# WWWindrunner/Cross-Modal-Video-Engine

Hardware: AMD Instinct MI355X
Metric: query-video pairs/sec scored + R@1/5/10 parity, MSR-VTT-1kA at 1/8 GPU (higher is better)
Workload: dtype f16

## Files before the change

cross-modal-video-engine_amd/csrc/cmve_internal.h:

```cpp
#pragma once
#include <hip/hip_runtime.h>
#include <hip/hip_ext.h>
#include <stdint.h>
#include <math.h>
#include <string>
#include <algorithm>
#include <type_traits>
#include "../../include/cmve.h"

struct cmve_handle {
  int device;
  hipStream_t stream;
  hipStream_t aux = nullptr;
  hipEvent_t ev[CMVE_MAX_CHUNKS + 2] = {};
  hipEvent_t tev[2 * CMVE_MAX_CHUNKS] = {};
  int last_chunks = 0;
  hipEvent_t eval_ev[CMVE_EVAL_TIMING_SLOTS][4] = {};
  hipEvent_t eval_kev[CMVE_EVAL_TIMING_SLOTS][8] = {};
  bool eval_no_fix[CMVE_EVAL_TIMING_SLOTS] = {};
  bool eval_chained[CMVE_EVAL_TIMING_SLOTS] = {};
  void* scratch = nullptr;
  size_t scratch_bytes = 0;
  void* comm = nullptr;
  int nranks = 1, rank = 0;
// ... 225 lines not shown
      load4d(x + k, v);
#pragma unroll
      for (int c = 0; c < 4; ++c) ss = fma(v[c], v[c], ss);
    }
    return wave_sum(ss);
  }
  for (int64_t k = lane; k < d; k += WAVE) {
    const double v = (double)x[k];
    ss = fma(v, v, ss);
  }
  return wave_sum(ss);
}
__device__ __forceinline__ double row_inv_norm(double ss, double eps, int flags) {
  const double nrm = sqrt(ss);
  return (flags & CMVE_PACK_RAW) ? 1.0 : (eps > 0.0 ? 1.0 / fmax(nrm, eps) : 1.0 / nrm);
}

struct PackAcc {
  double e1 = 0.0, e2 = 0.0, e3 = 0.0;
  float e4 = 0.f;
};

__device__ __forceinline__ int xcd_linear(int bid, int total) {
  const int xcd = bid & 7, local = bid >> 3;
  const int q = total >> 3, r = total & 7;
  return (xcd < r ? xcd * (q + 1) : r * (q + 1) + (xcd - r) * q) + local;
}

__device__ __forceinline__ uint16_t lo16_elem(float xf, _Float16 h, float& res) {
  const float d2 = xf - (float)h;
  const uint16_t lo = f2bf(d2);
  res = d2 - bf2f(lo);
  return lo;
}
__device__ __forceinline__ float lo16_bound(double ss_res) {
  return f32_round_up(sqrt(ss_res) * (1.0 + 1e-4) + 5.9605e-8 * (1.0 + 1e-6) + 1e-12);
}
__device__ __forceinline__ _Float16 f16_via_f32(double xh, float& xf) {
  xf = (float)xh;
  asm volatile("" : "+v"(xf));
  return (_Float16)xf;
}

__device__ __forceinline__ void pack_elem(double xh, bool want_f16, uint16_t& h, uint16_t& l, uint16_t& f,
                                          PackAcc& acc) {
  float xf;
  const _Float16 hf16 = f16_via_f32(xh, xf);
  if (want_f16) {
    const double r3 = xh - (double)hf16;
    acc.e3 = fma(r3, r3, acc.e3);
    f = __builtin_bit_cast(uint16_t, hf16);
  }
  h = f2bf(xf);
  const float hf = bf2f(h);
  l = f2bf(xf - hf);
  const double r1 = xh - (double)hf;
  const double r2 = r1 - (double)bf2f(l);
  acc.e1 = fma(r1, r1, acc.e1);
  acc.e2 = fma(r2, r2, acc.e2);
}

typedef unsigned short cmve_u16x4 __attribute__((ext_vector_type(4)));
typedef uint32_t cmve_u32x2 __attribute__((ext_vector_type(2)));

__device__ __forceinline__ void pack_pad_row(uint16_t* hrow, uint16_t* lrow, uint16_t* frow, int64_t d_pad,
                                             int lane) {
  const cmve_u16x4 z = {0, 0, 0, 0};
  for (int64_t k = (int64_t)lane * 4; k < d_pad; k += 256) {
    gst((cmve_u16x4*)(hrow + k), z);
    if (lrow) gst((cmve_u16x4*)(lrow + k), z);
    if (frow) gst((cmve_u16x4*)(frow + k), z);
  }
}

template <typename T>
__device__ __forceinline__ void pack_row_planes(const T* __restrict__ x, int64_t d, int64_t d_pad, bool vec,
                                                double inv, uint16_t* hrow, uint16_t* lrow, uint16_t* frow,
                                                int lane, float& b1, float& b2, float& b3) {
  const bool want_f16 = frow != nullptr;
  PackAcc acc;
  bool done = false;
  if (vec) {
    for (int64_t k = (int64_t)lane * 4; k < d_pad; k += 256) {
      cmve_u16x4 hv = {0, 0, 0, 0}, lv = {0, 0, 0, 0}, fv = {0, 0, 0, 0};
      if (k < d) {
        double e[4];
        load4d(x + k, e);
#pragma unroll
        for (int c = 0; c < 4; ++c) {
          uint16_t h, l, f = 0;
          pack_elem(e[c] * inv, want_f16, h, l, f, acc);
          hv[c] = h;
          lv[c] = l;
          fv[c] = f;
        }
      }
      *(cmve_u16x4*)(hrow + k) = hv;
      if (lrow) *(cmve_u16x4*)(lrow + k) = lv;
      if (frow) *(cmve_u16x4*)(frow + k) = fv;
    }
    done = true;
  }
  if (!done)
    for (int64_t k = lane; k < d_pad; k += WAVE) {
      uint16_t h = 0, l = 0, f = 0;
      if (k < d) pack_elem((double)x[k] * inv, want_f16, h, l, f, acc);
      hrow[k] = h;
      if (lrow) lrow[k] = l;
      if (frow) frow[k] = f;
    }
  const double e1 = wave_sum(acc.e1), e2 = wave_sum(acc.e2), e3 = wave_sum(acc.e3);
  b1 = f32_round_up(sqrt(e1) * (1.0 + 1e-9) + 1e-12);
  b2 = f32_round_up(sqrt(e2) * (1.0 + 1e-9) + 1e-12);
  b3 = f32_round_up(sqrt(e3) * (1.0 + 1e-9) + 1e-12);
}

__device__ __forceinline__ int64_t gt_rank_of(int32_t cnt, double sgt, int64_t n_m) {
  return (sgt != sgt) ? n_m + 1 : (sgt == (double)INFINITY ? n_m : (int64_t)cnt + 1);
}

constexpr int CAND_BUCKET_SHIFT = 8;
struct CandLayout {
  int64_t nb, cap_b;
};
inline CandLayout cand_layout(int64_t g_n_pad, int64_t cap) {
  CandLayout l;
  l.nb = std::max<int64_t>(1, (g_n_pad + (1 << CAND_BUCKET_SHIFT) - 1) >> CAND_BUCKET_SHIFT);
  l.cap_b = cap > l.nb ? (cap - l.nb) / l.nb : 0;
  return l;
}
constexpr int64_t FIXUP_MAX_BUCKETS_PER_XCD = 4096;
constexpr int EVAL_EMAX_SHARDS = 64;

template <typename TA, typename TB, bool LIGHT = false>
__device__ __forceinline__ double wave_cos64(const TA* xa, const TB* xb, double inva, double invb, int64_t d,
                                             int lane) {
  return wave_dot64<TA, TB, LIGHT>(xa, xb, d, lane) * (inva * invb);
}

typedef uint32_t cmve_u32x4 __attribute__((ext_vector_type(4)));
struct L16Frag {
  cmve_u32x4 h0, h1, l0, l1;
};
__device__ __forceinline__ void l16_load(const uint16_t* __restrict__ hrow, const uint16_t* __restrict__ lrow,
                                         int64_t k, L16Frag& f) {
  f.h0 = gld((const cmve_u32x4*)(hrow + k));
  f.h1 = gld((const cmve_u32x4*)(hrow + k + 8));
  f.l0 = gld((const cmve_u32x4*)(lrow + k));
  f.l1 = gld((const cmve_u32x4*)(lrow + k + 8));
}
__device__ __forceinline__ double l16_x(uint32_t hw, uint32_t lw, int half) {
  const uint16_t h = (uint16_t)(hw >> (16 * half));
  const uint32_t l = half ? (lw & 0xffff0000u) : (lw << 16);
  return (double)(float)__builtin_bit_cast(_Float16, h) + (double)__uint_as_float(l);
}
__device__ __forceinline__ double l16_partial(const L16Frag& a, const L16Frag& b, double acc) {
  const uint32_t ah[8] = {a.h0.x, a.h0.y, a.h0.z, a.h0.w, a.h1.x, a.h1.y, a.h1.z, a.h1.w};
  const uint32_t al[8] = {a.l0.x, a.l0.y, a.l0.z, a.l0.w, a.l1.x, a.l1.y, a.l1.z, a.l1.w};
  const uint32_t bh[8] = {b.h0.x, b.h0.y, b.h0.z, b.h0.w, b.h1.x, b.h1.y, b.h1.z, b.h1.w};
  const uint32_t bl[8] = {b.l0.x, b.l0.y, b.l0.z, b.l0.w, b.l1.x, b.l1.y, b.l1.z, b.l1.w};
#pragma unroll
  for (int e = 0; e < 16; ++e)
    acc = fma(l16_x(ah[e >> 1], al[e >> 1], e & 1), l16_x(bh[e >> 1], bl[e >> 1], e & 1), acc);
  return acc;
}
__device__ __forceinline__ void fixup_prefix(const uint64_t* __restrict__ cand, int64_t nb, int64_t cap_b, int xcd,
                                             int G, int64_t nk, int lane, int64_t* pre) {
  const int64_t per = (nk + 63) / 64;
  const int64_t k0 = lane * per, k1 = min(nk, k0 + per);
  if (per <= 4) {
    int64_t v[4];
#pragma unroll
    for (int j = 0; j < 4; ++j) v[j] = (k0 + j < k1) ? min((int64_t)gld(cand + xcd + G * (k0 + j)), cap_b) : 0;
    const int64_t sum = (v[0] + v[1]) + (v[2] + v[3]);
    int64_t incl = sum;
    for (int o = 1; o < 64; o <<= 1) {
      const int64_t t = __shfl_up(incl, o, 64);
      if (lane >= o) incl += t;
    }
    int64_t run = incl - sum;
#pragma unroll
    for (int j = 0; j < 4; ++j)
      if (k0 + j < k1) {
        pre[k0 + j] = run;
        run += v[j];
      }
    if (lane == 63) pre[nk] = incl;
  } else {
    int64_t sum = 0;
    for (int64_t k = k0; k < k1; ++k) sum += min((int64_t)gld(cand + xcd + G * k), cap_b);
    int64_t incl = sum;
    for (int o = 1; o < 64; o <<= 1) {
      const int64_t t = __shfl_up(incl, o, 64);
      if (lane >= o) incl += t;
    }
    int64_t run = incl - sum;
    for (int64_t k = k0; k < k1; ++k) {
      pre[k] = run;
      run += min((int64_t)gld(cand + xcd + G * k), cap_b);
    }
    if (lane == 63) pre[nk] = incl;
  }
}

template <typename TQ, typename TG, bool PREFETCH = false, bool DYN_PRE = false, bool LIGHT = false>
__device__ __forceinline__ void fixup_walk(const TQ* __restrict__ qraw, int64_t ldq,
                                                    const double* __restrict__ qinv, const TG* __restrict__ graw,
                                                    int64_t ldg, const double* __restrict__ ginv, int64_t d,
                                                    const double* __restrict__ row_sgt,
                                                    const double* __restrict__ col_sgt, int* __restrict__ row_cnt,
                                                    int* __restrict__ col_cnt, const uint64_t* __restrict__ cand,
                                                    int64_t nb, int64_t cap_b, bool flat = false) {
  int64_t* pre;
  if constexpr (DYN_PRE) {
    extern __shared__ int64_t fix_dyn_pre[];
    pre = fix_dyn_pre;
  } else {
    __shared__ int64_t fix_pre[FIXUP_MAX_BUCKETS_PER_XCD + 1];
    pre = fix_pre;
  }
  const int lane = threadIdx.x & 63, wave = threadIdx.x >> 6;
  const int G = flat ? 1 : 8;
  const int xcd = flat ? 0 : (blockIdx.x & 7);
  const int64_t nk = xcd < nb ? (nb - xcd + G - 1) / G : 0;
  if (wave == 0) fixup_prefix(cand, nb, cap_b, xcd, G, nk, lane, pre);
  __syncthreads();
  const int64_t total = pre[nk];
  const int nw = (int)(blockDim.x >> 6);
  const int64_t stride = (int64_t)(gridDim.x / G) * nw;
  int64_t k = 0;
  auto entry = [&](int64_t cc) -> uint64_t {
    if (cc >= total) return 0ull;
    if (pre[k + 1] <= cc) {
      int64_t lo = k + 1, hi = nk - 1;
      while (lo < hi) {
        const int64_t mid = (lo + hi + 1) >> 1;
        if (pre[mid] <= cc) lo = mid;
        else hi = mid - 1;
      }
      k = lo;
    }
    return gld(cand + nb + (xcd + G * k) * cap_b + (cc - pre[k]));
  };
  const int64_t c0 = (int64_t)(blockIdx.x / G) * nw + wave;
  uint64_t u_next = entry(c0);
  for (int64_t c = c0; c < total;) {
    const uint64_t u = u_next;
    c += stride;
    u_next = entry(c);
    const int64_t i = (int64_t)(u & 0x7fffffffull);
    const int64_t j = (int64_t)((u >> 31) & 0x7fffffffull);
    uint32_t flags = (uint32_t)(u >> 62);
    if (!flags) continue;
    double rs = 0.0, cs = 0.0;
    if (PREFETCH) {
      rs = ((flags & 1u) && row_sgt) ? gld(row_sgt + i) : 0.0;
      cs = ((flags & 2u) && col_sgt) ? gld(col_sgt + j) : 0.0;
    }
    const double s = wave_cos64<TQ, TG, LIGHT>(qraw + i * ldq, graw + j * ldg, gld(qinv + i), gld(ginv + j), d, lane);
    if (lane == 0) {
      if ((flags & 1u) && row_sgt && s > (PREFETCH ? rs : gld(row_sgt + i))) gadd(row_cnt + i, 1);
      if ((flags & 2u) && col_sgt && s > (PREFETCH ? cs : gld(col_sgt + j))) gadd(col_cnt + j, 1);
    }
  }
}

__device__ __forceinline__ uint32_t topk_key(float f) {
  const uint32_t u = __float_as_uint(f);
  if (f != f) return 0u;
  return (u & 0x80000000u) ? ~u : (u | 0x80000000u);
}
__device__ __forceinline__ float topk_key_inv(uint32_t k) {
  return __uint_as_float((k & 0x80000000u) ? (k & 0x7fffffffu) : ~k);
}

__host__ __device__ __forceinline__ double score_error_bound(double ea, double eb, int64_t d_pad, int mode) {
  const double n = (double)d_pad * (33.0 / 32.0) * (mode == CMVE_SIM_BF16X3 ? 3.0 : 1.0);
  const double u = 1.0 / 8388608.0;
  const double gamma = n * u / (1.0 - n * u);
  return ea + (1.0 + ea) * eb + gamma * (1.0 + ea) * (1.0 + eb) + 1e-12;
}

inline const float* mode_err(const cmve_rows_t* r, int mode) {
  return mode == CMVE_SIM_BF16 ? r->err_hi : (mode == CMVE_SIM_BF16X3 ? r->err_hilo : r->err_h16);
}
__host__ __device__ __forceinline__ int mode_slot(int mode) { return mode; }

}
```

cross-modal-video-engine_amd/csrc/sim.hip:

```cpp
#include <algorithm>
#include <vector>

#include <hip/hip_ext.h>

#include "cmve_internal.h"

#ifndef CMVE_SIM_GN
#define CMVE_SIM_GN 8
#endif
#ifndef CMVE_EVAL_DBG
#define CMVE_EVAL_DBG 0
#endif
namespace cmve {

typedef __bf16 bf16x8_t __attribute__((ext_vector_type(8)));
typedef _Float16 f16x8_t __attribute__((ext_vector_type(8)));
typedef short s16x8_t __attribute__((ext_vector_type(8)));
typedef float f32x4_t __attribute__((ext_vector_type(4)));
typedef __attribute__((address_space(3))) void lds_void_t;

constexpr int BK = 64;
constexpr int EPI_STORE = 0, EPI_RANK = 1, EPI_LINEAR = 2, EPI_TOPK = 3, EPI_BIAS = 4;
constexpr bool epi_thr(int e) { return e == EPI_RANK || e == EPI_TOPK; }

struct SimArgs {
  const uint16_t* qhi;
  const uint16_t* qlo;
  const uint16_t* ghi;
  const uint16_t* glo;
  int64_t ldk;
  int nq, ng;
  int nblk_m, nblk_n;
  int nk;
  int nk0;
  int gn;
  const float* bias;
  const float* bn_scale;
  const float* bn_shift;
  const float* resid;
  int64_t ldr;
  int relu;
  void* out;
  int64_t ldo;
  float alpha, beta;
  int out_f64;
  const float* row_hi;
  const float* row_lo;
  const float* col_hi;
  const float* col_lo;
  int* row_cnt;
  int* col_cnt;
  unsigned long long* cand;
  long long cand_cap;
  unsigned long long* cand_count;
  unsigned long long* bucket_cnt;
  long long cap_b;
  int thr_gt;
  const double* row_sgt;
  const double* col_sgt;
  const float* q_err;
  const float* g_err;
  const unsigned* q_emax;
  const unsigned* g_emax;
  unsigned long long* dbg_stamps;
  int tile_buckets;
  int nbn64;
  const int* row_gt1;
  const int* col_gt1;
  int fix_inline;
  int q_f64, g_f64;
  const void* q_raw;
  const void* g_raw;
  int64_t q_ld, g_ld, d;
  const double* q_inv;
  const double* g_inv;
  const uint16_t* q_lo16;
  const uint16_t* g_lo16;
  const float* q_el;
  const float* g_el;
  unsigned* l3_count;
  unsigned long long* l3;
  int l3_cap;
};

__device__ __forceinline__ void tile_grouped(int L, int nblk_m, int nblk_n, int GN, int& bm, int& bn);
__device__ __forceinline__ void tile_of_block(int bid, int nblk_m, int nblk_n, int GN, int& bm, int& bn) {
  tile_grouped(xcd_linear(bid, nblk_m * nblk_n), nblk_m, nblk_n, GN, bm, bn);
}
__device__ __forceinline__ void tile_grouped(int L, int nblk_m, int nblk_n, int GN, int& bm, int& bn) {
  const int group = L / (GN * nblk_m);
  const int within = L - group * (GN * nblk_m);
  const int gn = min(GN, nblk_n - group * GN);
  bm = within / gn;
  bn = group * GN + (within - bm * gn);
}

__host__ __device__ constexpr int lds_swz(int r) { return r & 7; }

__device__ __forceinline__ uint32_t stage_lane_off(int64_t ldk, int lane) {
  constexpr int CPR = BK / 8;
  const int r = lane / CPR, c = lane % CPR;
  return (uint32_t)(((int64_t)r * ldk + (c ^ lds_swz(r)) * 8) * 2);
}

template <int ROWS, int NW>
__device__ __forceinline__ void stage_plane(const uint16_t* __restrict__ src, int64_t ldk, int row0, int k0,
                                            char* lds_plane, int wave, uint32_t loff) {
  constexpr int RPI = 64 / (BK / 8);
  constexpr int PER_WAVE = ROWS / RPI / NW;
  static_assert(PER_WAVE * RPI * NW == ROWS, "plane rows must split evenly over the waves");
  static_assert(lds_swz(RPI) == 0 && lds_swz(RPI - 1) == lds_swz(2 * RPI - 1), "swizzle period");
  const char* blk = (const char*)(src + ((int64_t)row0 + wave * PER_WAVE * RPI) * ldk + k0);
#pragma unroll
  for (int it = 0; it < PER_WAVE; ++it)
    __builtin_amdgcn_global_load_lds((const void*)(blk + (int64_t)it * RPI * ldk * 2 + loff),
                                     (lds_void_t*)(lds_plane + (wave * PER_WAVE + it) * 1024), 16, 0, 0);
}

__device__ __forceinline__ s16x8_t read_frag(const char* plane, int row, int chunk) {
  return *(const s16x8_t*)(plane + row * (BK * 2) + ((chunk ^ lds_swz(row)) << 4));
}

__device__ __forceinline__ void lds_add_u32_async(int* p, int v) {
  const uint32_t addr = (uint32_t)(uintptr_t)(__attribute__((address_space(3))) int*)p;
  asm volatile("ds_add_u32 %0, %1" ::"v"(addr), "v"(v) : "memory");
}

__device__ __forceinline__ uint32_t row_sum16(uint32_t v) {
  v += (uint32_t)__builtin_amdgcn_update_dpp(0, (int)v, 0xB1, 0xF, 0xF, false);
  v += (uint32_t)__builtin_amdgcn_update_dpp(0, (int)v, 0x4E, 0xF, 0xF, false);
  v += (uint32_t)__builtin_amdgcn_update_dpp(0, (int)v, 0x141, 0xF, 0xF, false);
  v += (uint32_t)__builtin_amdgcn_update_dpp(0, (int)v, 0x140, 0xF, 0xF, false);
  return v;
}

template <int R>
__device__ __forceinline__ uint32_t row4_count_bits(float s0, float s1, float s2, float s3, float hi, float lo,
                                                    uint32_t& u) {
  uint32_t c, b0, b1, b2, b3;
  unsigned long long m0, m1, m2, m3, l0, l1, l2, l3, cc;
  asm("v_cmp_gt_f32_e64 %[m0], %[s0], %[hi]\n\t"
      "v_cmp_gt_f32_e64 %[m1], %[s1], %[hi]\n\t"
      "v_cmp_gt_f32_e64 %[m2], %[s2], %[hi]\n\t"
      "v_cmp_gt_f32_e64 %[m3], %[s3], %[hi]\n\t"
      "v_cmp_ge_f32_e64 %[l0], %[s0], %[lo]\n\t"
      "v_cmp_ge_f32_e64 %[l1], %[s1], %[lo]\n\t"
      "v_cmp_ge_f32_e64 %[l2], %[s2], %[lo]\n\t"
      "v_cmp_ge_f32_e64 %[l3], %[s3], %[lo]\n\t"
      "v_cndmask_b32_e64 %[c], 0, 1, %[m0]\n\t"
      "v_addc_co_u32_e64 %[c], %[cc], %[c], 0, %[m1]\n\t"
      "v_addc_co_u32_e64 %[c], %[cc], %[c], 0, %[m2]\n\t"
      "v_addc_co_u32_e64 %[c], %[cc], %[c], 0, %[m3]\n\t"
      "s_andn2_b64 %[l0], %[l0], %[m0]\n\t"
      "s_andn2_b64 %[l1], %[l1], %[m1]\n\t"
      "s_andn2_b64 %[l2], %[l2], %[m2]\n\t"
      "s_andn2_b64 %[l3], %[l3], %[m3]\n\t"
      "v_cndmask_b32_e64 %[b0], 0, 1, %[l0]\n\t"
      "v_cndmask_b32_e64 %[b1], 0, 1, %[l1]\n\t"
      "v_cndmask_b32_e64 %[b2], 0, 1, %[l2]\n\t"
      "v_cndmask_b32_e64 %[b3], 0, 1, %[l3]\n\t"
      "v_lshl_or_b32 %[u], %[b0], %[sh0], %[u]\n\t"
      "v_lshl_or_b32 %[u], %[b1], %[sh1], %[u]\n\t"
      "v_lshl_or_b32 %[u], %[b2], %[sh2], %[u]\n\t"
      "v_lshl_or_b32 %[u], %[b3], %[sh3], %[u]"
      : [c] "=&v"(c), [b0] "=&v"(b0), [b1] "=&v"(b1), [b2] "=&v"(b2), [b3] "=&v"(b3), [u] "+v"(u),
        [m0] "=&s"(m0), [m1] "=&s"(m1), [m2] "=&s"(m2), [m3] "=&s"(m3), [l0] "=&s"(l0), [l1] "=&s"(l1),
        [l2] "=&s"(l2), [l3] "=&s"(l3), [cc] "=&s"(cc)
      : [s0] "v"(s0), [s1] "v"(s1), [s2] "v"(s2), [s3] "v"(s3), [hi] "v"(hi), [lo] "v"(lo), [sh0] "n"(R),
        [sh1] "n"(4 + R), [sh2] "n"(8 + R), [sh3] "n"(12 + R));
  return c;
}

__device__ __forceinline__ void pair2_count_bits(float sa, float sb, float hia, float loa, float hib, float lob,
                                                 float chi, float clo, uint32_t& ca, uint32_t& cb, uint32_t& cc,
                                                 uint32_t& urow, uint32_t& ucol) {
  unsigned long long ma, mb, na, nb, la, lb, ka, kb, cy;
  asm("v_cmp_gt_f32_e64 %[ma], %[sa], %[hia]\n\t"
      "v_cmp_gt_f32_e64 %[mb], %[sb], %[hib]\n\t"
      "v_cmp_gt_f32_e64 %[na], %[sa], %[chi]\n\t"
      "v_cmp_gt_f32_e64 %[nb], %[sb], %[chi]\n\t"
      "v_cmp_ge_f32_e64 %[la], %[sa], %[loa]\n\t"
      "v_cmp_ge_f32_e64 %[lb], %[sb], %[lob]\n\t"
      "v_cmp_ge_f32_e64 %[ka], %[sa], %[clo]\n\t"
      "v_cmp_ge_f32_e64 %[kb], %[sb], %[clo]\n\t"
      "v_addc_co_u32_e64 %[ca], %[cy], %[ca], 0, %[ma]\n\t"
      "v_addc_co_u32_e64 %[cb], %[cy], %[cb], 0, %[mb]\n\t"
      "v_addc_co_u32_e64 %[cc], %[cy], %[cc], 0, %[na]\n\t"
      "v_addc_co_u32_e64 %[cc], %[cy], %[cc], 0, %[nb]\n\t"
      "s_andn2_b64 %[la], %[la], %[ma]\n\t"
      "s_andn2_b64 %[lb], %[lb], %[mb]\n\t"
      "s_andn2_b64 %[ka], %[ka], %[na]\n\t"
      "s_andn2_b64 %[kb], %[kb], %[nb]\n\t"
      "v_addc_co_u32_e64 %[ur], %[cy], %[ur], %[ur], %[la]\n\t"
      "v_addc_co_u32_e64 %[ur], %[cy], %[ur], %[ur], %[lb]\n\t"
      "v_addc_co_u32_e64 %[uc], %[cy], %[uc], %[uc], %[ka]\n\t"
      "v_addc_co_u32_e64 %[uc], %[cy], %[uc], %[uc], %[kb]"
      : [ca] "+v"(ca), [cb] "+v"(cb), [cc] "+v"(cc), [ur] "+v"(urow), [uc] "+v"(ucol), [ma] "=&s"(ma),
        [mb] "=&s"(mb), [na] "=&s"(na), [nb] "=&s"(nb), [la] "=&s"(la), [lb] "=&s"(lb), [ka] "=&s"(ka),
        [kb] "=&s"(kb), [cy] "=&s"(cy)
      : [sa] "v"(sa), [sb] "v"(sb), [hia] "v"(hia), [loa] "v"(loa), [hib] "v"(hib), [lob] "v"(lob), [chi] "v"(chi),
        [clo] "v"(clo));
}

template <int MODE>
__device__ __forceinline__ f32x4_t mfma(s16x8_t a, s16x8_t b, f32x4_t c) {
  if constexpr (MODE == CMVE_SIM_F16)
    return __builtin_amdgcn_mfma_f32_16x16x32_f16(__builtin_bit_cast(f16x8_t, a), __builtin_bit_cast(f16x8_t, b), c,
                                                  0, 0, 0);
  else
    return __builtin_amdgcn_mfma_f32_16x16x32_bf16(__builtin_bit_cast(bf16x8_t, a), __builtin_bit_cast(bf16x8_t, b),
                                                   c, 0, 0, 0);
}

template <int WM, int WN, int TM>
struct Geo {
  static constexpr int TN = 4;
  static constexpr int NW = WM * WN;
  static constexpr int NT = NW * 64;
  static constexpr int BM = WM * TM * 16;
  static constexpr int BN = WN * TN * 16;
};

template <int MODE, int BM, int BN, bool PHASED>
constexpr size_t stage_bytes() {
  return (size_t)((MODE == CMVE_SIM_BF16X3 && !PHASED) ? 2 : 1) * (BM + BN) * BK * 2;
}

template <int BM, int BN, bool PHASED>
constexpr bool is_ring() {
  return !PHASED && BN == 64 && (BM == 64 || BM == 128);
}

#ifndef CMVE_G64_STAGES
#define CMVE_G64_STAGES 4
#endif
#ifndef CMVE_G128R_STAGES
#define CMVE_G128R_STAGES 2
#endif
template <int BM, int BN, bool PHASED>
constexpr int ring_stages() {
  return !is_ring<BM, BN, PHASED>() ? 2 : (BM == 64 ? CMVE_G64_STAGES : CMVE_G128R_STAGES);
}

template <int MODE, int BM, int BN, bool PHASED>
constexpr size_t ring_lds_bytes() {
  return ring_stages<BM, BN, PHASED>() * stage_bytes<MODE, BM, BN, PHASED>();
}

#ifdef CMVE_DBG_STAMPS
#define CMVE_STAMP(k) \
  if (threadIdx.x == 0) a.bucket_cnt[(size_t)tile * 8 + (k)] = __builtin_amdgcn_s_memtime()
#else
#define CMVE_STAMP(k) \
  if constexpr (!PHASED) {  \
    if (a.dbg_stamps && threadIdx.x == 0) gst(a.dbg_stamps + (size_t)tile * 8 + (k), __builtin_amdgcn_s_memrealtime()); \
  }
#endif

__device__ __forceinline__ void plane_of(int tp, bool& a_lo, bool& b_lo, int& kt) {
  kt = tp / 3;
  const int p = tp - 3 * kt;
  a_lo = p == 0;
  b_lo = p == 1;
}

#define CMVE_BAR_LDS() asm volatile("s_waitcnt lgkmcnt(0)\n\ts_barrier" ::: "memory")

#ifndef CMVE_INL_LIST
#define CMVE_INL_LIST 1024
#endif
template <int BM, int BN, bool RANK, bool INL = false>
struct EpiLds {
  int rc[BM];
  int cc[BN];
  float thr[2 * (BM + BN)];
  double sgt[INL ? BM + BN : 1];
  uint32_t list[INL ? CMVE_INL_LIST : 1];
  int wtot[INL ? 16 : 1];
};
template <int BM, int BN, bool INL>
// ... 312 lines not shown
                ccnt[j] += sc[r] > chi[j];
                hit |= __builtin_amdgcn_fmed3f(sc[r], clo[j], chi[j]) == sc[r];
              }
            }
          }
          if constexpr (DR) row_reduce(i, c0 | (c1 << 8) | (c2 << 16) | (c3 << 24));
          und[i] = __builtin_amdgcn_ballot_w64(hit) ? und_bits(i, rhi, rlo, DR, DC) : 0u;
          } else {
          uint32_t u = 0u;
          if constexpr (DR && DC && TN == 4) {
            uint32_t ur = 0u, uc = 0u;
  #pragma unroll
            for (int j = TN - 1; j >= 0; --j) {
              pair2_count_bits(acc[i][j][3], acc[i][j][2], rhi[3], rlo[3], rhi[2], rlo[2], chi[j], clo[j], c3, c2,
                               ccnt[j], ur, uc);
              pair2_count_bits(acc[i][j][1], acc[i][j][0], rhi[1], rlo[1], rhi[0], rlo[0], chi[j], clo[j], c1, c0,
                               ccnt[j], ur, uc);
            }
            row_reduce(i, c0 | (c1 << 8) | (c2 << 16) | (c3 << 24));
            und[i] = ur | (uc << 16);
            continue;
          }
          if constexpr (DR && !DC && TN == 4) {
            c0 = row4_count_bits<0>(acc[i][0][0], acc[i][1][0], acc[i][2][0], acc[i][3][0], rhi[0], rlo[0], u);
            c1 = row4_count_bits<1>(acc[i][0][1], acc[i][1][1], acc[i][2][1], acc[i][3][1], rhi[1], rlo[1], u);
            c2 = row4_count_bits<2>(acc[i][0][2], acc[i][1][2], acc[i][2][2], acc[i][3][2], rhi[2], rlo[2], u);
            c3 = row4_count_bits<3>(acc[i][0][3], acc[i][1][3], acc[i][2][3], acc[i][3][3], rhi[3], rlo[3], u);
            row_reduce(i, c0 | (c1 << 8) | (c2 << 16) | (c3 << 24));
            und[i] = u;
            continue;
          }
  #pragma unroll
          for (int j = 0; j < TN; ++j) {
            const f32x4_t sc = acc[i][j];
            if constexpr (DR) {
              c0 += sc[0] > rhi[0];
              c1 += sc[1] > rhi[1];
              c2 += sc[2] > rhi[2];
              c3 += sc[3] > rhi[3];
  #pragma unroll
              for (int r = 0; r < 4; ++r) u |= (sc[r] >= rlo[r] && sc[r] <= rhi[r]) ? (1u << (j * 4 + r)) : 0u;
            }
            if constexpr (DC) {
  #pragma unroll
              for (int r = 0; r < 4; ++r) {
                ccnt[j] += sc[r] > chi[j];
                u |= (sc[r] >= clo[j] && sc[r] <= chi[j]) ? (1u << (16 + j * 4 + r)) : 0u;
              }
            }
          }
          if constexpr (DR) row_reduce(i, c0 | (c1 << 8) | (c2 << 16) | (c3 << 24));
          und[i] = u;
          }
        }
        if constexpr (DC) {
  #pragma unroll
          for (int j = 0; j < TN; ++j) cc_pack += ccnt[j] << (8 * j);
        }
      };
      if (padded) {
              for (int i = 0; i < TM; ++i)
#pragma unroll
          for (int j = 0; j < TN; ++j)
#pragma unroll
            for (int r = 0; r < 4; ++r)
              if (!((rowok >> (i * 4 + r)) & (colok >> j) & 1u)) acc[i][j][r] = -INFINITY;
      }
      if (KG > 1 && group != 0) {
#pragma unroll
        for (int i = 0; i < TM; ++i) und[i] = 0u;
      } else if (do_row && do_col) {
        fast_block(std::true_type{}, std::true_type{});
      } else if (do_row) {
        fast_block(std::true_type{}, std::false_type{});
      } else {
        fast_block(std::false_type{}, std::true_type{});
      }
      if constexpr (GT_SKIP) {
#pragma unroll
        for (int i = 0; i < TM; ++i) {
          uint32_t m = 0u;
#pragma unroll
          for (int r = 0; r < 4; ++r) {
            const int dc = gt_row[i][r] - cbase;
            m |= (dc >= 0 && dc < TN * 16 && (dc & 15) == 0) ? 1u << ((dc >> 4) * 4 + r) : 0u;
          }
#pragma unroll
          for (int j = 0; j < TN; ++j) {
            const int dr = gt_col[j] - (rbase + i * 16);
            m |= (dr >= 0 && dr < 4) ? 1u << (16 + j * 4 + dr) : 0u;
          }
          und[i] &= ~m;
        }
      }
      cc_pack += __shfl_xor(cc_pack, 16, 64);
      cc_pack += __shfl_xor(cc_pack, 32, 64);
      if (lane < 16) {
  #pragma unroll
        for (int j = 0; j < TN; ++j) {
          const uint32_t c = (cc_pack >> (8 * j)) & 0xffu;
          if (c) lds_add_u32_async(&lds_cc[wc * (TN * 16) + j * 16 + lane], (int)c);
        }
      }
      CMVE_STAMP(5);
      uint32_t nmine = 0u;
  #pragma unroll
      for (int i = 0; i < TM; ++i) nmine += __builtin_popcount((und[i] | (und[i] >> 16)) & 0xffffu);
      uint32_t excl = 0u, total = 0u;
      if (__builtin_amdgcn_ballot_w64(nmine != 0u)) {
  #pragma unroll
        for (int b = 0; b < 8; ++b) {
          const unsigned long long m = __builtin_amdgcn_ballot_w64((nmine >> b) & 1u);
          excl += __builtin_amdgcn_mbcnt_hi((uint32_t)(m >> 32), __builtin_amdgcn_mbcnt_lo((uint32_t)m, 0u)) << b;
          total += (uint32_t)__builtin_popcountll(m) << b;
        }
      }
      const int bucket = EPI == EPI_TOPK ? (m0 >> 8)
                                         : (a.tile_buckets ? (m0 >> 6) * a.nbn64 + (n0 >> 6) : (n0 >> CAND_BUCKET_SHIFT));
      unsigned long long wbase = 0ull;
      bool inl = false;
      if constexpr (INL) inl = a.fix_inline != 0;
      if (total && lane == 0 && !inl) wbase = gadd(a.bucket_cnt + bucket, (unsigned long long)total);
      if constexpr (INL) {
        if (a.fix_inline) {
          if (lane == 0) epi.wtot[wave] = (int)total;
          CMVE_BAR_LDS();
          int woff = 0, ntot = 0;
#pragma unroll
          for (int w = 0; w < NWT; ++w) {
            const int t = epi.wtot[w];
            woff += w < wave ? t : 0;
            ntot += t;
          }
          bool listed = ntot <= CMVE_INL_LIST;
          if (listed && nmine) {
            uint32_t slot = (uint32_t)woff + excl;
#pragma unroll
            for (int i = 0; i < TM; ++i) {
              uint32_t m = (und[i] | (und[i] >> 16)) & 0xffffu;
              while (m) {
                const int bit = __builtin_ctz(m);
                m &= m - 1u;
                const uint32_t lr = (uint32_t)(rbase - m0 + i * 16 + (bit & 3));
                const uint32_t lc = (uint32_t)(cbase - n0 + (bit >> 2) * 16);
                const uint32_t fl = ((und[i] >> bit) & 1u) | (((und[i] >> (16 + bit)) & 1u) << 1);
                epi.list[slot++] = lr | (lc << 8) | (fl << 16);
              }
            }
          }
          if (listed) {
            CMVE_BAR_LDS();
            if (a.q_lo16) {
              struct L2Stage {
                uint32_t ent;
                int64_t qr, gc;
                float elq, elg;
                L16Frag fq, fg;
              };
              auto l2_fetch = [&](int p, L2Stage& st) {
                st.ent = epi.list[p];
                st.qr = m0 + (st.ent & 0xff);
                st.gc = n0 + ((st.ent >> 8) & 0xff);
                st.elq = gld(a.q_el + st.qr);
                st.elg = gld(a.g_el + st.gc);
                const int64_t k = 16 * (int64_t)lane;
                if (k < a.ldk) {
                  l16_load(a.qhi + st.qr * a.ldk, a.q_lo16 + st.qr * a.ldk, k, st.fq);
                  l16_load(a.ghi + st.gc * a.ldk, a.g_lo16 + st.gc * a.ldk, k, st.fg);
                }
              };
              auto l2_finish = [&](int p, const L2Stage& st) {
                double s2 = 16 * (int64_t)lane < a.ldk ? l16_partial(st.fq, st.fg, 0.0) : 0.0;
#pragma unroll
                for (int o = 32; o >= 1; o >>= 1) s2 += __shfl_xor(s2, o, 64);
                if (lane == 0) {
                  const double eq = (double)st.elq, eg = (double)st.elg;
                  const double E2 = eq + (1.0 + eq) * eg + 2e-12;
                  uint32_t fl = (st.ent >> 16) & 3u;
                  const int lr = (int)(st.ent & 0xff), lc = (int)((st.ent >> 8) & 0xff);
                  if (fl & 1u) {
                    const double t = epi.sgt[lr];
                    if (s2 - E2 > t) { lds_add_u32_async(&lds_rc[lr], 1); fl &= ~1u; }
                    else if (s2 + E2 < t) fl &= ~1u;
                  }
                  if (fl & 2u) {
                    const double t = epi.sgt[BM + lc];
                    if (s2 - E2 > t) { lds_add_u32_async(&lds_cc[lc], 1); fl &= ~2u; }
                    else if (s2 + E2 < t) fl &= ~2u;
                  }
                  if (fl && a.l3_count) {
                    const unsigned slot = gadd(a.l3_count, 1u);
                    if (a.l3 && slot < (unsigned)a.l3_cap) {
                      gst(a.l3 + slot, (unsigned long long)st.qr | ((unsigned long long)st.gc << 31) |
                                           ((unsigned long long)fl << 62));
                      fl = 0u;
                    }
                  }
                  epi.list[p] = (st.ent & 0xffffu) | (fl << 16);
                }
              };
              {
                L2Stage sa, sb;
                int p = wave;
                if (p < ntot) l2_fetch(p, sa);
                while (p < ntot) {
                  int pn = p + NWT;
                  if (pn < ntot) l2_fetch(pn, sb);
                  l2_finish(p, sa);
                  p = pn;
                  if (p >= ntot) break;
                  pn = p + NWT;
                  if (pn < ntot) l2_fetch(pn, sa);
                  l2_finish(p, sb);
                  p = pn;
                }
              }
              CMVE_BAR_LDS();
            }
            auto rescore2 = [&](uint32_t e1, uint32_t e2, bool two) {
              const int64_t r1 = m0 + (e1 & 0xff), c1 = n0 + ((e1 >> 8) & 0xff);
              const int64_t r2 = two ? m0 + (e2 & 0xff) : r1, c2 = two ? n0 + ((e2 >> 8) & 0xff) : c1;
              const double inv1 = gld(a.q_inv + r1) * gld(a.g_inv + c1), inv2 = gld(a.q_inv + r2) * gld(a.g_inv + c2);
              double d1, d2;
              if (a.q_f64) {
                const double* q = (const double*)a.q_raw;
                if (a.g_f64) {
                  const double* g = (const double*)a.g_raw;
                  wave_dot64_x2(q + r1 * a.q_ld, g + c1 * a.g_ld, q + r2 * a.q_ld, g + c2 * a.g_ld, a.d, lane, d1, d2);
                } else {
                  const float* g = (const float*)a.g_raw;
                  wave_dot64_x2(q + r1 * a.q_ld, g + c1 * a.g_ld, q + r2 * a.q_ld, g + c2 * a.g_ld, a.d, lane, d1, d2);
                }
              } else {
                const float* q = (const float*)a.q_raw;
                if (a.g_f64) {
                  const double* g = (const double*)a.g_raw;
                  wave_dot64_x2(q + r1 * a.q_ld, g + c1 * a.g_ld, q + r2 * a.q_ld, g + c2 * a.g_ld, a.d, lane, d1, d2);
                } else {
                  const float* g = (const float*)a.g_raw;
                  wave_dot64_x2(q + r1 * a.q_ld, g + c1 * a.g_ld, q + r2 * a.q_ld, g + c2 * a.g_ld, a.d, lane, d1, d2);
                }
              }
              if (lane == 0) {
                const double s1 = d1 * inv1;
                if ((e1 >> 16) & 1u) { if (s1 > epi.sgt[r1 - m0]) lds_add_u32_async(&lds_rc[r1 - m0], 1); }
                if ((e1 >> 17) & 1u) { if (s1 > epi.sgt[BM + c1 - n0]) lds_add_u32_async(&lds_cc[c1 - n0], 1); }
                if (two) {
                  const double s2 = d2 * inv2;
                  if ((e2 >> 16) & 1u) { if (s2 > epi.sgt[r2 - m0]) lds_add_u32_async(&lds_rc[r2 - m0], 1); }
                  if ((e2 >> 17) & 1u) { if (s2 > epi.sgt[BM + c2 - n0]) lds_add_u32_async(&lds_cc[c2 - n0], 1); }
                }
              }
            };
            if constexpr (BATCH) {
              for (int p = wave; p < ntot; p += NWT) {
                const uint32_t e = epi.list[p];
                if (!(e >> 16)) continue;
                const int64_t r1 = m0 + (e & 0xff), c1 = n0 + ((e >> 8) & 0xff);
                const double inva = gld(a.q_inv + r1), invb = gld(a.g_inv + c1);
                double s1;
                if (a.q_f64) {
                  const double* x = (const double*)a.q_raw + r1 * a.q_ld;
                  s1 = a.g_f64 ? wave_cos64(x, (const double*)a.g_raw + c1 * a.g_ld, inva, invb, a.d, lane)
                               : wave_cos64(x, (const float*)a.g_raw + c1 * a.g_ld, inva, invb, a.d, lane);
                } else {
                  const float* x = (const float*)a.q_raw + r1 * a.q_ld;
                  s1 = a.g_f64 ? wave_cos64(x, (const double*)a.g_raw + c1 * a.g_ld, inva, invb, a.d, lane)
                               : wave_cos64(x, (const float*)a.g_raw + c1 * a.g_ld, inva, invb, a.d, lane);
                }
                if (lane == 0) {
                  if ((e >> 16) & 1u) { if (s1 > epi.sgt[r1 - m0]) lds_add_u32_async(&lds_rc[r1 - m0], 1); }
                  if ((e >> 17) & 1u) { if (s1 > epi.sgt[BM + c1 - n0]) lds_add_u32_async(&lds_cc[c1 - n0], 1); }
                }
              }
            } else if (a.q_lo16) {
              for (int p = wave; p < ntot; p += NWT) {
                const uint32_t e = epi.list[p];
                if (e >> 16) rescore2(e, 0u, false);
              }
            } else {
              for (int p = 2 * wave; p < ntot; p += 2 * NWT)
                rescore2(epi.list[p], p + 1 < ntot ? epi.list[p + 1] : 0u, p + 1 < ntot);
            }
          } else {
#pragma unroll
            for (int i = 0; i < TM; ++i) {
              uint32_t bits = (und[i] | (und[i] >> 16)) & 0xffffu;
              unsigned long long m;
              while ((m = __builtin_amdgcn_ballot_w64(bits != 0u))) {
                const int src = (int)__builtin_ctzll(m);
                const uint32_t sb = (uint32_t)__builtin_amdgcn_readlane((int)bits, src);
                const uint32_t su = (uint32_t)__builtin_amdgcn_readlane((int)und[i], src);
                const int bit = __builtin_ctz(sb);
                if (lane == src) bits &= bits - 1u;
                const int lr = wr * (TM * 16) + (src >> 4) * 4 + i * 16 + (bit & 3);
                const int lc = wc * (TN * 16) + (src & 15) + (bit >> 2) * 16;
                const int64_t row = m0 + lr, col = n0 + lc;
                const double inva = gld(a.q_inv + row), invb = gld(a.g_inv + col);
                double sc;
                if (a.q_f64) {
                  const double* x = (const double*)a.q_raw + row * a.q_ld;
                  sc = a.g_f64 ? wave_cos64(x, (const double*)a.g_raw + col * a.g_ld, inva, invb, a.d, lane)
                               : wave_cos64(x, (const float*)a.g_raw + col * a.g_ld, inva, invb, a.d, lane);
                } else {
                  const float* x = (const float*)a.q_raw + row * a.q_ld;
                  sc = a.g_f64 ? wave_cos64(x, (const double*)a.g_raw + col * a.g_ld, inva, invb, a.d, lane)
                               : wave_cos64(x, (const float*)a.g_raw + col * a.g_ld, inva, invb, a.d, lane);
                }
                if (lane == 0) {
                  if (((su >> bit) & 1u) && sc > epi.sgt[lr]) lds_add_u32_async(&lds_rc[lr], 1);
                  if (((su >> (16 + bit)) & 1u) && sc > epi.sgt[BM + lc]) lds_add_u32_async(&lds_cc[lc], 1);
                }
              }
            }
          }
        }
      }
      CMVE_STAMP(6);
      CMVE_BAR_LDS();
      for (int t = tid; t < BM + BN; t += NTT) {
        const int c = lds_rc[t];
        lds_rc[t] = 0;
        if (!c) continue;
        if (t < BM) {
          if (a.row_cnt && m0 + t < a.nq) gadd(a.row_cnt + m0 + t, c);
        } else {
          if (a.col_cnt && n0 + t - BM < a.ng) gadd(a.col_cnt + n0 + t - BM, c);
        }
      }
      if (inl && total && lane == 0) gadd(a.bucket_cnt + bucket, (unsigned long long)total);
      const bool emit = total != 0u && !inl;
      if (emit) {
        const unsigned long long w0 = __shfl(wbase, 0, 64);
        unsigned long long slot = w0 + excl;
        unsigned long long* dst = a.cand + (size_t)bucket * a.cap_b;
  #pragma unroll
        for (int i = 0; i < TM; ++i) {
          uint32_t m = (und[i] | (und[i] >> 16)) & 0xffffu;
          while (m) {
            const int bit = __builtin_ctz(m);
            m &= m - 1u;
            unsigned long long packed;
            if constexpr (EPI == EPI_TOPK) {
              float sc = acc[i][0][0];
  #pragma unroll
              for (int jj = 0; jj < TN; ++jj)
  #pragma unroll
                for (int r = 0; r < 4; ++r) sc = (bit == jj * 4 + r) ? acc[i][jj][r] : sc;
              packed = ((unsigned long long)topk_key(sc) << 32) |
                       ((unsigned long long)((rbase + i * 16 + (bit & 3)) & 255) << 24) |
                       (unsigned long long)(cbase + (bit >> 2) * 16);
            } else {
              const unsigned long long flags = ((und[i] >> bit) & 1u) | (((und[i] >> (16 + bit)) & 1u) << 1);
              packed = (unsigned long long)(rbase + i * 16 + (bit & 3)) |
                       ((unsigned long long)(cbase + (bit >> 2) * 16) << 31) | (flags << 62);
            }
            if ((long long)slot < a.cap_b) gst(dst + slot, packed);
            ++slot;
          }
        }
      }
  #ifdef CMVE_DBG_STAMPS
      CMVE_BAR_LDS();
  #endif
      CMVE_STAMP(3);
    }
  };

  const int frow = lane & 15;
// ... 1297 lines not shown
```

Baseline: 135.5 billion.

## Restructure level-2 rescoring: DPP wave reduction, LDS staging, block-parallel decisions

The level-2 precise rescoring pass now computes each pair's dot product with two independent FMA chains and sums in float before widening to double. The cross-lane reduction uses DPP and permlane swaps in place of a shuffle-xor ladder. Lane 0 writes each score and its error terms as a 128-bit record into LDS that aliases the staging ring. A separate block-wide pass then runs the threshold decisions one entry per thread and uses a ballot plus a single atomic per wave for level-3 overflow slots, replacing the serial lane-0 decisions and per-entry atomics. Costs are an extra barrier, reliance on ring LDS capacity, and slightly different rounding in the hi+lo reconstruction.

Result: faster. 140.2 billion, median of 6 (+3.4%).

```diff
diff --git a/cross-modal-video-engine_amd/csrc/cmve_internal.h b/cross-modal-video-engine_amd/csrc/cmve_internal.h
--- a/cross-modal-video-engine_amd/csrc/cmve_internal.h
+++ b/cross-modal-video-engine_amd/csrc/cmve_internal.h
@@ -401,17 +401,50 @@
 __device__ __forceinline__ double l16_x(uint32_t hw, uint32_t lw, int half) {
   const uint16_t h = (uint16_t)(hw >> (16 * half));
   const uint32_t l = half ? (lw & 0xffff0000u) : (lw << 16);
-  return (double)(float)__builtin_bit_cast(_Float16, h) + (double)__uint_as_float(l);
-}
-__device__ __forceinline__ double l16_partial(const L16Frag& a, const L16Frag& b, double acc) {
+  return (double)((float)__builtin_bit_cast(_Float16, h) + __uint_as_float(l));
+}
+__device__ __forceinline__ double l16_partial(const L16Frag& a, const L16Frag& b) {
   const uint32_t ah[8] = {a.h0.x, a.h0.y, a.h0.z, a.h0.w, a.h1.x, a.h1.y, a.h1.z, a.h1.w};
   const uint32_t al[8] = {a.l0.x, a.l0.y, a.l0.z, a.l0.w, a.l1.x, a.l1.y, a.l1.z, a.l1.w};
   const uint32_t bh[8] = {b.h0.x, b.h0.y, b.h0.z, b.h0.w, b.h1.x, b.h1.y, b.h1.z, b.h1.w};
   const uint32_t bl[8] = {b.l0.x, b.l0.y, b.l0.z, b.l0.w, b.l1.x, b.l1.y, b.l1.z, b.l1.w};
-#pragma unroll
-  for (int e = 0; e < 16; ++e)
-    acc = fma(l16_x(ah[e >> 1], al[e >> 1], e & 1), l16_x(bh[e >> 1], bl[e >> 1], e & 1), acc);
-  return acc;
+  double acc0 = 0.0, acc1 = 0.0;
+#pragma unroll
+  for (int w = 0; w < 8; ++w) {
+    acc0 = fma(l16_x(ah[w], al[w], 0), l16_x(bh[w], bl[w], 0), acc0);
+    acc1 = fma(l16_x(ah[w], al[w], 1), l16_x(bh[w], bl[w], 1), acc1);
+  }
+  return acc0 + acc1;
+}
+template <int CTRL>
+__device__ __forceinline__ double l16_dpp(double v) {
+  const uint64_t b = __builtin_bit_cast(uint64_t, v);
+  const uint32_t lo = (uint32_t)__builtin_amdgcn_update_dpp(0, (int)(uint32_t)b, CTRL, 0xF, 0xF, false);
+  const uint32_t hi = (uint32_t)__builtin_amdgcn_update_dpp(0, (int)(uint32_t)(b >> 32), CTRL, 0xF, 0xF, false);
+  return __builtin_bit_cast(double, (uint64_t)lo | ((uint64_t)hi << 32));
+}
+__device__ __forceinline__ double l16_wave_sum(double v) {
+  v += l16_dpp<0xB1>(v);
+  v += l16_dpp<0x4E>(v);
+  v += l16_dpp<0x141>(v);
+  v += l16_dpp<0x140>(v);
+  {
+    const uint64_t b = __builtin_bit_cast(uint64_t, v);
+    const uint32_t lo = (uint32_t)b, hi = (uint32_t)(b >> 32);
+    const auto sl = __builtin_amdgcn_permlane16_swap(lo, lo, false, false);
+    const auto sh = __builtin_amdgcn_permlane16_swap(hi, hi, false, false);
+    v = __builtin_bit_cast(double, (uint64_t)sl[0] | ((uint64_t)sh[0] << 32)) +
+        __builtin_bit_cast(double, (uint64_t)sl[1] | ((uint64_t)sh[1] << 32));
+  }
+  {
+    const uint64_t b = __builtin_bit_cast(uint64_t, v);
+    const uint32_t lo = (uint32_t)b, hi = (uint32_t)(b >> 32);
+    const auto sl = __builtin_amdgcn_permlane32_swap(lo, lo, false, false);
+    const auto sh = __builtin_amdgcn_permlane32_swap(hi, hi, false, false);
+    v = __builtin_bit_cast(double, (uint64_t)sl[0] | ((uint64_t)sh[0] << 32)) +
+        __builtin_bit_cast(double, (uint64_t)sl[1] | ((uint64_t)sh[1] << 32));
+  }
+  return v;
 }
 __device__ __forceinline__ void fixup_prefix(const uint64_t* __restrict__ cand, int64_t nb, int64_t cap_b, int xcd,
                                              int G, int64_t nk, int lane, int64_t* pre) {
diff --git a/cross-modal-video-engine_amd/csrc/sim.hip b/cross-modal-video-engine_amd/csrc/sim.hip
--- a/cross-modal-video-engine_amd/csrc/sim.hip
+++ b/cross-modal-video-engine_amd/csrc/sim.hip
@@ -126,6 +126,11 @@
   asm volatile("ds_add_u32 %0, %1" ::"v"(addr), "v"(v) : "memory");
 }
 
+__device__ __forceinline__ void lds_write_b128_async(void* p, cmve_u32x4 v) {
+  const uint32_t addr = (uint32_t)(uintptr_t)(__attribute__((address_space(3))) char*)p;
+  asm volatile("ds_write_b128 %0, %1" ::"v"(addr), "v"(v) : "memory");
+}
+
 __device__ __forceinline__ uint32_t row_sum16(uint32_t v) {
   v += (uint32_t)__builtin_amdgcn_update_dpp(0, (int)v, 0xB1, 0xF, 0xF, false);
   v += (uint32_t)__builtin_amdgcn_update_dpp(0, (int)v, 0x4E, 0xF, 0xF, false);
@@ -744,69 +749,94 @@
             CMVE_BAR_LDS();
             if (a.q_lo16) {
               struct L2Stage {
-                uint32_t ent;
-                int64_t qr, gc;
                 float elq, elg;
                 L16Frag fq, fg;
               };
+              static_assert(!INL || ring_lds_bytes<MODE, BM, BN, PHASED>() >= (size_t)CMVE_INL_LIST * 16,
+                            "the level-2 scores alias the staging ring");
+              const int64_t l2_ldk = a.ldk;
+              const bool l2_inrow = 16 * (int64_t)lane < l2_ldk;
+              const int64_t l2_k = l2_inrow ? 16 * (int64_t)lane : 0;
               auto l2_fetch = [&](int p, L2Stage& st) {
-                st.ent = epi.list[p];
-                st.qr = m0 + (st.ent & 0xff);
-                st.gc = n0 + ((st.ent >> 8) & 0xff);
-                st.elq = gld(a.q_el + st.qr);
-                st.elg = gld(a.g_el + st.gc);
-                const int64_t k = 16 * (int64_t)lane;
-                if (k < a.ldk) {
-                  l16_load(a.qhi + st.qr * a.ldk, a.q_lo16 + st.qr * a.ldk, k, st.fq);
-                  l16_load(a.ghi + st.gc * a.ldk, a.g_lo16 + st.gc * a.ldk, k, st.fg);
+                const uint32_t ent = epi.list[p];
+                const int64_t qr = m0 + (ent & 0xff), gc = n0 + ((ent >> 8) & 0xff);
+                st.elq = gld(a.q_el + qr);
+                st.elg = gld(a.g_el + gc);
+                l16_load(a.qhi + qr * l2_ldk, a.q_lo16 + qr * l2_ldk, l2_k, st.fq);
+                l16_load(a.ghi + gc * l2_ldk, a.g_lo16 + gc * l2_ldk, l2_k, st.fg);
+                __builtin_amdgcn_sched_barrier(0);
+              };
+              auto l2_finish = [&](int p, const L2Stage& st) {
+                const double part = l16_partial(st.fq, st.fg);
+                const double s2 = l16_wave_sum(l2_inrow ? part : 0.0);
+                if (lane == 0) {
+                  const uint64_t sb = __builtin_bit_cast(uint64_t, s2);
+                  const cmve_u32x4 rec = {(uint32_t)sb, (uint32_t)(sb >> 32), __float_as_uint(st.elq),
+                                          __float_as_uint(st.elg)};
+                  lds_write_b128_async(smem + 16 * p, rec);
                 }
               };
-              auto l2_finish = [&](int p, const L2Stage& st) {
-                double s2 = 16 * (int64_t)lane < a.ldk ? l16_partial(st.fq, st.fg, 0.0) : 0.0;
-#pragma unroll
-                for (int o = 32; o >= 1; o >>= 1) s2 += __shfl_xor(s2, o, 64);
-                if (lane == 0) {
-                  const double eq = (double)st.elq, eg = (double)st.elg;
-                  const double E2 = eq + (1.0 + eq) * eg + 2e-12;
-                  uint32_t fl = (st.ent >> 16) & 3u;
-                  const int lr = (int)(st.ent & 0xff), lc = (int)((st.ent >> 8) & 0xff);
-                  if (fl & 1u) {
-                    const double t = epi.sgt[lr];
-                    if (s2 - E2 > t) { lds_add_u32_async(&lds_rc[lr], 1); fl &= ~1u; }
-                    else if (s2 + E2 < t) fl &= ~1u;
-                  }
-                  if (fl & 2u) {
-                    const double t = epi.sgt[BM + lc];
-                    if (s2 - E2 > t) { lds_add_u32_async(&lds_cc[lc], 1); fl &= ~2u; }
-                    else if (s2 + E2 < t) fl &= ~2u;
-                  }
-                  if (fl && a.l3_count) {
-                    const unsigned slot = gadd(a.l3_count, 1u);
-                    if (a.l3 && slot < (unsigned)a.l3_cap) {
-                      gst(a.l3 + slot, (unsigned long long)st.qr | ((unsigned long long)st.gc << 31) |
-                                           ((unsigned long long)fl << 62));
-                      fl = 0u;
+              auto l2_decide = [&]() {
+                for (int t0 = 0; t0 < ntot; t0 += NTT) {
+                  const int t = t0 + tid;
+                  uint32_t ent = 0u, fl = 0u;
+                  if (t < ntot) {
+                    ent = epi.list[t];
+                    const cmve_u32x4 rec = *(const cmve_u32x4*)(smem + 16 * t);
+                    const double s2 = __builtin_bit_cast(double, (uint64_t)rec.x | ((uint64_t)rec.y << 32));
+                    const double eq = (double)__uint_as_float(rec.z), eg = (double)__uint_as_float(rec.w);
+                    const double E2 = eq + (1.0 + eq) * eg + 2e-12;
+                    fl = (ent >> 16) & 3u;
+                    const int lr = (int)(ent & 0xff), lc = (int)((ent >> 8) & 0xff);
+                    if (fl & 1u) {
+                      const double sg = epi.sgt[lr];
+                      if (s2 - E2 > sg) { lds_add_u32_async(&lds_rc[lr], 1); fl &= ~1u; }
+                      else if (s2 + E2 < sg) fl &= ~1u;
+                    }
+                    if (fl & 2u) {
+                      const double sg = epi.sgt[BM + lc];
+                      if (s2 - E2 > sg) { lds_add_u32_async(&lds_cc[lc], 1); fl &= ~2u; }
+                      else if (s2 + E2 < sg) fl &= ~2u;
                     }
                   }
-                  epi.list[p] = (st.ent & 0xffffu) | (fl << 16);
+                  if (a.l3_count) {
+                    const unsigned long long um = __builtin_amdgcn_ballot_w64(fl != 0u);
+                    if (um) {
+                      unsigned base = 0u;
+                      if (lane == 0) base = gadd(a.l3_count, (unsigned)__builtin_popcountll(um));
+                      base = (unsigned)__builtin_amdgcn_readfirstlane((int)base);
+                      const unsigned slot = base + __builtin_amdgcn_mbcnt_hi((uint32_t)(um >> 32),
+                                                                             __builtin_amdgcn_mbcnt_lo((uint32_t)um, 0u));
+                      if (fl && a.l3 && slot < (unsigned)a.l3_cap) {
+                        gst(a.l3 + slot, (unsigned long long)(m0 + (ent & 0xff)) |
+                                             ((unsigned long long)(n0 + ((ent >> 8) & 0xff)) << 31) |
+                                             ((unsigned long long)fl << 62));
+                        fl = 0u;
+                      }
+                    }
+                  }
+                  if (t < ntot) epi.list[t] = (ent & 0xffffu) | (fl << 16);
                 }
               };
               {
                 L2Stage sa, sb;
                 int p = wave;
-                if (p < ntot) l2_fetch(p, sa);
-                while (p < ntot) {
-                  int pn = p + NWT;
-                  if (pn < ntot) l2_fetch(pn, sb);
-                  l2_finish(p, sa);
-                  p = pn;
-                  if (p >= ntot) break;
-                  pn = p + NWT;
-                  if (pn < ntot) l2_fetch(pn, sa);
-                  l2_finish(p, sb);
-                  p = pn;
+                if (p < ntot) {
+                  l2_fetch(p, sa);
+                  for (;;) {
+                    if (p + NWT >= ntot) { l2_finish(p, sa); break; }
+                    l2_fetch(p + NWT, sb);
+                    l2_finish(p, sa);
+                    p += NWT;
+                    if (p + NWT >= ntot) { l2_finish(p, sb); break; }
+                    l2_fetch(p + NWT, sa);
+                    l2_finish(p, sb);
+                    p += NWT;
+                  }
                 }
               }
+              CMVE_BAR_LDS();
+              l2_decide();
               CMVE_BAR_LDS();
             }
             auto rescore2 = [&](uint32_t e1, uint32_t e2, bool two) {
```
